# EugenHotaj/pytorch-generative

Measured on NVIDIA H100. Metric: images/sec training step (ImageGPT CIFAR-10 32x32), higher is better.
Workload: dtype bf16

## Files before the change

pytorch_generative_b200/csrc/pg_common.cuh:

```cuda
#pragma once

#include <cuda.h>
#include <cuda_bf16.h>
#include <cuda_runtime.h>
#include <stdint.h>
#include <stdio.h>

#include "../../include/pg_b200.h"

typedef __nv_bfloat16 bf16;
typedef __nv_bfloat162 bf162;

void pg_set_error(const char* fmt, ...);
int pg_check_launch(const char* what);

#define PG_REQUIRE(cond, ...)            \
  do {                                   \
    if (!(cond)) {                       \
      pg_set_error(__VA_ARGS__);         \
      return 1;                          \
    }                                    \
  } while (0)

static inline bool pg_aligned16(const void* p) { return (reinterpret_cast<uintptr_t>(p) & 15) == 0; }

#define PG_CUDA(call)                                                             \
  do {                                                                            \
    cudaError_t _e = (call);                                                      \
    if (_e != cudaSuccess) {                                                      \
      pg_set_error("%s failed: %s (%s:%d)", #call, cudaGetErrorString(_e), __FILE__, __LINE__); \
      return 1;                                                                   \
    }                                                                             \
  } while (0)

int pg_make_tmap_2d_bf16(CUtensorMap* out, const void* base, uint64_t rows, uint64_t cols,
                         uint64_t ld, uint32_t box_rows, uint32_t box_cols);
int pg_make_tmap_nd_bf16(CUtensorMap* out, const void* base, int rank, const uint64_t* dims,
                         const uint64_t* strides_bytes , const uint32_t* box,
                         int swizzle128);
int pg_make_tmap_nd(CUtensorMap* out, const void* base, int elem_bytes, int rank, const uint64_t* dims,
                    const uint64_t* strides_bytes, const uint32_t* box, int swizzle_bytes);
int pg_make_tmap_2d(CUtensorMap* out, const void* base, int elem_bytes, uint64_t rows, uint64_t cols, uint64_t ld,
                    uint32_t box_rows, uint32_t box_cols, int swizzle_bytes);
int pg_num_sms();
int pg_scratch(size_t bytes, cudaStream_t stream, float** out);
int pg_sum_partials(const float* part, int nparts, long long part_stride, int M, int N, int64_t ld_out, float* out,
                    cudaStream_t stream);

#ifdef __CUDACC__

__device__ __forceinline__ uint32_t smem_u32(const void* p) {
  return static_cast<uint32_t>(__cvta_generic_to_shared(p));
}

__device__ __forceinline__ void mbar_init(uint64_t* bar, uint32_t count) {
  asm volatile("mbarrier.init.shared::cta.b64 [%0], %1;" ::"r"(smem_u32(bar)), "r"(count) : "memory");
}
__device__ __forceinline__ void fence_barrier_init() {
  asm volatile("fence.mbarrier_init.release.cluster;" ::: "memory");
}
__device__ __forceinline__ void fence_proxy_async_smem() {
  asm volatile("fence.proxy.async.shared::cta;" ::: "memory");
}
__device__ __forceinline__ void mbar_arrive_expect_tx(uint64_t* bar, uint32_t bytes) {
  asm volatile("mbarrier.arrive.expect_tx.shared::cta.b64 _, [%0], %1;" ::"r"(smem_u32(bar)), "r"(bytes)
               : "memory");
}
__device__ __forceinline__ void mbar_arrive(uint64_t* bar) {
  asm volatile("mbarrier.arrive.shared::cta.b64 _, [%0];" ::"r"(smem_u32(bar)) : "memory");
}
__device__ __forceinline__ bool mbar_try_wait(uint64_t* bar, uint32_t parity) {
  uint32_t ok;
  asm volatile(
      "{\n\t.reg .pred p;\n\t"
      "mbarrier.try_wait.parity.shared::cta.b64 p, [%1], %2;\n\t"
      "selp.u32 %0, 1, 0, p;\n\t}"
      : "=r"(ok)
      : "r"(smem_u32(bar)), "r"(parity)
      : "memory");
  return ok != 0;
// ... 238 lines not shown
```

pytorch_generative_b200/csrc/pg_gemm.cu:

```cuda
#include <stdlib.h>
#include <string.h>

#include "../../include/pg_b200.h"
#include "pg_common.cuh"

namespace {

constexpr int BM = 128;
constexpr int BK = 64;
constexpr int A_STAGE_BYTES = BM * BK * 2;
constexpr int SMEM_LIMIT = 232448;

constexpr int MAX_CONV_TAPS = 225;
struct ConvGeom {
  int mode, H, W, C, T;
  int cslabs;
  int nbpt;
  int8_t dy[MAX_CONV_TAPS], dx[MAX_CONV_TAPS];
};

struct GemmParams {
  ConvGeom conv;
  int M, N, K;
  int num_m_blk, num_n_blk;
  int k_iters;
  int k_per_split;
  int splits;
  int stages;
  int epi_tma, epi_nbuf, epi_buf_bytes, epi_in_bytes;
  int off_old, off_res0, off_res1, off_aux, off_f32, off_pre, off_bf16;
  int epi_smem;
  int store_deriv;
  int res_bf16;
  float* a_rowsum;
  float* split_part;
  float* rowsum_part;
  pg_gemm_epilogue epi;
};

struct EpiMaps {
  CUtensorMap res0, res1, aux, out_f32, out_pre, out_bf16;
  CUtensorMap bias;
};

template <bool BWD, int ACT, int N>
__device__ __forceinline__ void act_as(float (&x)[N]) {
#pragma unroll
  for (int i = 0; i < N; ++i) x[i] = BWD ? pg_act_bwd(ACT, x[i]) : pg_act_fwd(ACT, x[i]);
}
template <bool BWD, int N>
__device__ __forceinline__ void act_n(int act, float (&x)[N]) {
  switch (act) {
    case PG_ACT_RELU: act_as<BWD, PG_ACT_RELU>(x); break;
    case PG_ACT_GELU: act_as<BWD, PG_ACT_GELU>(x); break;
    case PG_ACT_ELU: act_as<BWD, PG_ACT_ELU>(x); break;
    case PG_ACT_TANH: act_as<BWD, PG_ACT_TANH>(x); break;
    case PG_ACT_GIVEN: act_as<BWD, PG_ACT_GIVEN>(x); break;
    case PG_ACT_RELU_OUT: act_as<BWD, PG_ACT_RELU_OUT>(x); break;
    case PG_ACT_ELU_OUT: act_as<BWD, PG_ACT_ELU_OUT>(x); break;
    default: act_as<BWD, PG_ACT_NONE>(x); break;
  }
}

__device__ __forceinline__ void epilogue_row32(const GemmParams& p, int row, int col0, int ncols, bool first_split,
                                               const uint32_t (&acc)[32], float* out_f32, int64_t ld_out_f32,
                                               bool accumulate) {
  const pg_gemm_epilogue& e = p.epi;
// ... 23 lines not shown
    float* o = out_f32 + (size_t)row * ld_out_f32 + col0;
    if (accumulate) {
      for (int i = 0; i < ncols; ++i) o[i] += v[i];
    } else {
      for (int i = 0; i < ncols; ++i) o[i] = v[i];
    }
  }
  if (e.out_pre) {
    bf16* o = reinterpret_cast<bf16*>(e.out_pre) + (size_t)row * e.ld_out_pre + col0;
    float d[32];
#pragma unroll
    for (int i = 0; i < 32; ++i) d[i] = v[i];
    if (p.store_deriv) act_n<true>(e.act, d);
    for (int i = 0; i < ncols; ++i) o[i] = __float2bfloat16(d[i]);
  }
  if (e.out_bf16) {
    bf16* o = reinterpret_cast<bf16*>(e.out_bf16) + (size_t)row * e.ld_out_bf16 + col0;
    if (e.act != PG_ACT_NONE) act_n<false>(e.act, v);
    for (int i = 0; i < ncols; ++i) o[i] = __float2bfloat16(v[i]);
  }
}

constexpr int GEMM_THREADS = 384;
constexpr int XP_LD = 68;
constexpr int XP_BYTES = 64 * XP_LD * 4;
constexpr int MAX_STAGES = 8;
constexpr int MAX_EPI_BUFS = 4;
constexpr int EPI_F32_BYTES = 16 * 32 * 4;
constexpr int EPI_BF16_BYTES = 16 * 32 * 2;
constexpr int EPI_BIAS_BYTES = 128 * 4;
constexpr int PRODUCER_REGS = 56;
constexpr int CONSUMER_REGS = 224;
constexpr uint32_t XPOSE_BAR = 1;
constexpr uint32_t ROWSUM_BAR = 3;
constexpr uint32_t MMA_TURN_BAR = 4;

struct WorkItem {
  int m_blk, n_blk, ks, k0, k1;
};
__device__ __forceinline__ WorkItem work_item(const GemmParams& p, int tile) {
  WorkItem w;
  w.n_blk = tile % p.num_n_blk;
  const int rest = tile / p.num_n_blk;
  w.m_blk = rest % p.num_m_blk;
  w.ks = rest / p.num_m_blk;
  w.k0 = w.ks * p.k_per_split;
  w.k1 = min(w.k0 + p.k_per_split, p.k_iters);
  return w;
}

template <int BN, bool A_MN, bool B_MN>
__device__ __forceinline__ void consumer_mainloop(uint8_t* smem, uint64_t* full_bar, uint64_t* empty_bar, int stages,
                                                  const WorkItem& w, int& s, uint32_t& ph, float (&acc)[2][BN / 2],
                                                  int turn_bar) {
  constexpr int STAGE_BYTES = A_STAGE_BYTES + BN * BK * 2;
  const int lane = threadIdx.x & 31;
  int prev = -1;
  for (int kit = w.k0; kit < w.k1; ++kit) {
    mbar_wait(&full_bar[s], ph);
    const uint32_t a_addr = smem_u32(smem + s * STAGE_BYTES);
    const uint32_t b_addr = smem_u32(smem + s * STAGE_BYTES) + A_STAGE_BYTES;
    const uint64_t b_base = B_MN ? wgmma_desc_sw128(b_addr, BK * 128, 1024) : wgmma_desc_sw128(b_addr, 16, 1024);
    wgmma_fence();
#pragma unroll
    for (int kk = 0; kk < BK / 16; ++kk) {
#pragma unroll
      for (int sl = 0; sl < 2; ++sl) {
// ... 256 lines not shown
        if (f32_out) tma_store_3d(&tm.out_f32, buf + p.off_f32, col, row, w.ks);
        if (pre_out) tma_store_2d(&tm.out_pre, buf + p.off_pre, col, row);
        if (bf16_out) tma_store_2d(&tm.out_bf16, buf + p.off_bf16, col, row);
      }
      bulk_commit_group();
      if (has_in) {
        bulk_wait_group_read<1>();
        if (i + nb - 1 < NSUB) epi_load<BN>(p, tm, w, r, g0, i + nb - 1);
      } else if (nb == 4) {
        bulk_wait_group_read<3>();
      } else if (nb == 3) {
        bulk_wait_group_read<2>();
      } else {
        bulk_wait_group_read<1>();
      }
    }
    if (++b == nb) { b = 0; par ^= 1u; }
  }
}

template <int BN, bool A_MN, bool B_MN, int EK>
__global__ void __launch_bounds__(GEMM_THREADS, 1)
gemm_wgmma_kernel(const __grid_constant__ CUtensorMap tmA, const __grid_constant__ CUtensorMap tmB,
                  const __grid_constant__ EpiMaps tmE, const GemmParams p) {
  constexpr int STAGE_BYTES = A_STAGE_BYTES + BN * BK * 2;
  extern __shared__ uint8_t smem_raw[];
  uint8_t* smem = smem_raw + ((1024u - (smem_u32(smem_raw) & 1023u)) & 1023u);
  const int STAGES = p.stages;
  uint8_t* const epi = smem + STAGES * STAGE_BYTES;
  uint64_t* full_bar = reinterpret_cast<uint64_t*>(epi + p.epi_smem);
  uint64_t* empty_bar = full_bar + MAX_STAGES;
  uint64_t* in_bar = empty_bar + MAX_STAGES;
  uint64_t* bias_bar = in_bar + 8 * MAX_EPI_BUFS;
  float* rowsum_xch = reinterpret_cast<float*>(bias_bar + 2);

  const int warp = threadIdx.x >> 5;
  const int lane = threadIdx.x & 31;
  const bool rowsum = A_MN && p.a_rowsum != nullptr;
  const int num_tiles = p.num_m_blk * p.num_n_blk * p.splits;
  if (threadIdx.x == 0) {
    tma_prefetch_desc(&tmA);
    tma_prefetch_desc(&tmB);
    for (int i = 0; i < STAGES; ++i) {
      mbar_init(&full_bar[i], 1);
      mbar_init(&empty_bar[i], rowsum ? 6 : 4);
    }
    for (int i = 0; i < 8 * MAX_EPI_BUFS + 2; ++i) mbar_init(&in_bar[i], 1);
    fence_barrier_init();
    fence_proxy_async_smem();
  }
  __syncthreads();

  if (warp < 4) {
    setmaxnreg_dec<PRODUCER_REGS>();
    if (warp == 0) {
      int s = 0;
      uint32_t ph = 0;
      for (int tile = blockIdx.x; tile < num_tiles; tile += gridDim.x) {
        const WorkItem w = work_item(p, tile);
        const int m_blk = w.m_blk, n_blk = w.n_blk;
        for (int kit = w.k0; kit < w.k1; ++kit) {
          mbar_wait(&empty_bar[s], ph ^ 1);
          uint8_t* sA = smem + s * STAGE_BYTES;
          uint8_t* sB = sA + A_STAGE_BYTES;
          mbar_arrive_expect_tx_w(&full_bar[s], STAGE_BYTES);
          if (p.conv.mode != 0) {
            const int hw = p.conv.H * p.conv.W;
// ... 10 lines not shown
              }
            } else {
              const int t = n_blk / p.conv.nbpt, nb = n_blk - t * p.conv.nbpt;
              const int pix0 = kit * BK, n = pix0 / hw, h0 = (pix0 - n * hw) / p.conv.W;
#pragma unroll
              for (int j = 0; j < BM / 64; ++j)
                tma_load_2d_w(sA + j * (BK * 128), &tmA, &full_bar[s], m_blk * BM + j * 64, kit * BK);
#pragma unroll
              for (int j = 0; j < BN / 64; ++j)
                tma_load_4d_w(sB + j * (BK * 128), &tmB, &full_bar[s], nb * BN + j * 64, p.conv.dx[t], h0 + p.conv.dy[t], n);
            }
          } else {
            if (!A_MN) {
              tma_load_2d_w(sA, &tmA, &full_bar[s], kit * BK, m_blk * BM);
            } else {
#pragma unroll
              for (int j = 0; j < BM / 64; ++j)
                tma_load_2d_w(sA + j * (BK * 128), &tmA, &full_bar[s], m_blk * BM + j * 64, kit * BK);
            }
            if (!B_MN) {
              tma_load_2d_w(sB, &tmB, &full_bar[s], kit * BK, n_blk * BN);
            } else {
#pragma unroll
              for (int j = 0; j < BN / 64; ++j)
                tma_load_2d_w(sB + j * (BK * 128), &tmB, &full_bar[s], n_blk * BN + j * 64, kit * BK);
            }
          }
          if (++s == STAGES) { s = 0; ph ^= 1; }
        }
      }
    } else if (A_MN && (warp == 2 || warp == 3)) {
      if (rowsum) {
        const int t = (warp - 2) * 32 + lane;
        const int c = t & 15, g = t >> 4;
        const uint32_t atom = (uint32_t)(c >> 3) * (BK * 128), cc = (uint32_t)(c & 7);
        int s = 0;
        uint32_t ph = 0;
        for (int tile = blockIdx.x; tile < num_tiles; tile += gridDim.x) {
          const WorkItem w = work_item(p, tile);
          const bool mine = (w.n_blk == 0);
          float acc[8];
#pragma unroll
          for (int q = 0; q < 8; ++q) acc[q] = 0.f;
          for (int kit = w.k0; kit < w.k1; ++kit) {
            mbar_wait(&full_bar[s], ph);
            if (mine) {
              const uint8_t* sA = smem + s * STAGE_BYTES + atom;
#pragma unroll
              for (int i = 0; i < BK / 4; ++i) {
                const uint32_t k = (uint32_t)(g + 4 * i);
                const uint4 v = *reinterpret_cast<const uint4*>(sA + k * 128 + ((cc ^ (k & 7u)) << 4));
                const uint32_t ww[4] = {v.x, v.y, v.z, v.w};
#pragma unroll
                for (int j = 0; j < 4; ++j) {
                  const float2 f = unpack_bf16x2(ww[j]);
                  acc[2 * j] += f.x;
                  acc[2 * j + 1] += f.y;
                }
              }
            }
            __syncwarp();
            if (lane == 0) mbar_arrive(&empty_bar[s]);
            if (++s == STAGES) { s = 0; ph ^= 1; }
          }
          if (mine) {
#pragma unroll
            for (int q = 0; q < 8; ++q) acc[q] += __shfl_xor_sync(0xffffffffu, acc[q], 16);
            named_bar_sync(ROWSUM_BAR, 64);
            if (warp == 3 && lane < 16) {
#pragma unroll
              for (int q = 0; q < 8; ++q) rowsum_xch[lane * 8 + q] = acc[q];
            }
            named_bar_sync(ROWSUM_BAR, 64);
            if (warp == 2 && lane < 16) {
#pragma unroll
              for (int q = 0; q < 8; ++q) acc[q] += rowsum_xch[lane * 8 + q];
              const int m0 = w.m_blk * BM + c * 8;
#pragma unroll
              for (int q = 0; q < 8; ++q)
                if (m0 + q < p.M) {
                  if (p.rowsum_part) p.rowsum_part[(size_t)w.ks * p.M + m0 + q] = acc[q];
                  else p.a_rowsum[m0 + q] += acc[q];
                }
            }
          }
        }
      }
    }
  } else {
    setmaxnreg_inc<CONSUMER_REGS>();
    const int cw = (warp - 4) >> 2;
    float* const xp = reinterpret_cast<float*>(epi) + cw * 64 * XP_LD;
    float acc[2][BN / 2];
    int s = 0;
    uint32_t ph = 0;
    int i = 0;
    for (int tile = blockIdx.x; tile < num_tiles; tile += gridDim.x, ++i) {
      const WorkItem w = work_item(p, tile);
      if ((i & 1) != cw) {
        const int pos = s + (w.k1 - w.k0);
        ph ^= (uint32_t)((pos / STAGES) & 1);
        s = pos % STAGES;
        continue;
      }
      const bool has_next = tile + (int)gridDim.x < num_tiles;
      if (p.epi_tma) epi_prologue<BN>(p, tmE, w, epi_ring(p, epi, cw), i >> 1);
      if (i > 0) named_bar_sync(MMA_TURN_BAR + cw, 256);
      if (p.epi_tma) epi_bias<BN>(p, tmE, w, epi_ring(p, epi, cw));
      consumer_mainloop<BN, A_MN, B_MN>(smem, full_bar, empty_bar, STAGES, w, s, ph, acc,
                                        has_next ? (int)(MMA_TURN_BAR + (cw ^ 1)) : -1);
      if constexpr (BN <= 64) {
        if (!p.epi_tma) consumer_epilogue<BN>(p, w, acc, xp, XPOSE_BAR + cw);
      }
      if (p.epi_tma) {
        const EpiRing r = epi_ring(p, epi, cw);
        if constexpr (EK != EK_GENERIC)
// ... 85 lines not shown
    if (e.bias) t += e.bias[n];
    if (p.res_bf16) {
      if (e.res0) t += __bfloat162float(reinterpret_cast<const bf16*>(e.res0)[(size_t)m * e.ld_res + n]);
      if (e.res1) t += __bfloat162float(reinterpret_cast<const bf16*>(e.res1)[(size_t)m * e.ld_res + n]);
    } else {
      if (e.res0) t += e.res0[(size_t)m * e.ld_res + n];
      if (e.res1) t += e.res1[(size_t)m * e.ld_res + n];
    }
    if (e.out_f32) e.out_f32[(size_t)m * e.ld_out_f32 + n] = t;
    if (e.out_pre)
      reinterpret_cast<bf16*>(e.out_pre)[(size_t)m * e.ld_out_pre + n] =
          __float2bfloat16(p.store_deriv ? pg_act_bwd(e.act, t) : t);
    if (e.out_bf16) reinterpret_cast<bf16*>(e.out_bf16)[(size_t)m * e.ld_out_bf16 + n] = __float2bfloat16(pg_act_fwd(e.act, t));
  }
}

int epi_kind(const GemmParams& p) {
  const pg_gemm_epilogue& e = p.epi;
  if (!p.epi_tma || e.alpha != 1.f || p.res_bf16 || p.off_old >= 0 || p.splits > 1) return EK_GENERIC;
  const bool bias = e.bias != nullptr, f32 = e.out_f32 != nullptr, bf = e.out_bf16 != nullptr;
  const bool pre = e.out_pre != nullptr, res0 = e.res0 != nullptr, res1 = e.res1 != nullptr;
  const bool no_act = e.act == PG_ACT_NONE && !p.store_deriv;
  if (bf && !f32 && !pre && !res0 && !res1 && no_act && e.dact == PG_ACT_NONE) return bias ? EK_BIAS_BF16 : EK_PLAIN;
  if (bf && !f32 && !pre && !res0 && !res1 && no_act && e.dact == PG_ACT_GIVEN && !bias) return EK_GIVEN_BF16;
  if (bf && pre && !f32 && !res0 && !res1 && bias && e.act == PG_ACT_GELU && p.store_deriv && e.dact == PG_ACT_NONE)
    return EK_BIAS_GELU2;
  if (f32 && !bf && !pre && res0 && bias && no_act && e.dact == PG_ACT_NONE)
    return res1 ? EK_BIAS_RES2_F32 : EK_BIAS_RES_F32;
  return EK_GENERIC;
}

template <int BN, bool A_MN, bool B_MN>
int launch_tc(const void* A, int64_t lda, const void* B, int64_t ldb, GemmParams& p, cudaStream_t stream) {
  CUtensorMap tmA, tmB;
  const ConvGeom& cg = p.conv;
  auto conv_map = [&](CUtensorMap* out, const void* base, int64_t ld, int pixels_per_box) {
    const int64_t n_img = (cg.mode == 1 ? (int64_t)p.M : (int64_t)p.K) / ((int64_t)cg.H * cg.W);
    uint64_t dims[4] = {(uint64_t)cg.C, (uint64_t)cg.W, (uint64_t)cg.H, (uint64_t)n_img};
    uint64_t strides[3] = {(uint64_t)ld * 2, (uint64_t)cg.W * ld * 2, (uint64_t)cg.H * cg.W * ld * 2};
    uint32_t box[4] = {64, (uint32_t)cg.W, (uint32_t)(pixels_per_box / cg.W), 1};
    return pg_make_tmap_nd_bf16(out, base, 4, dims, strides, box, 1);
  };
  if (cg.mode == 1) {
    if (conv_map(&tmA, A, lda, BM)) return 1;
  } else if (!A_MN) {
    if (pg_make_tmap_2d_bf16(&tmA, A, p.M, p.K, lda, BM, BK)) return 1;
  } else {
    if (pg_make_tmap_2d_bf16(&tmA, A, p.K, p.M, lda, BK, 64)) return 1;
  }
  if (cg.mode == 2) {
    PG_REQUIRE(B_MN && cg.C % BN == 0, "pg_gemm_bf16_conv(wgrad): channels (%d) must be a multiple of the N tile (%d)", cg.C, BN);
    p.conv.nbpt = cg.C / BN;
    if (conv_map(&tmB, B, ldb, BK)) return 1;
  } else if (!B_MN) {
    if (pg_make_tmap_2d_bf16(&tmB, B, p.N, p.K, ldb, BN, BK)) return 1;
  } else if (cg.mode == 1) {
    if (pg_make_tmap_2d_bf16(&tmB, B, cg.C, (uint64_t)cg.T * p.N, ldb, BK, 64)) return 1;
  } else {
    if (pg_make_tmap_2d_bf16(&tmB, B, p.K, p.N, ldb, BK, 64)) return 1;
  }
  EpiMaps tmE;
  memset(&tmE, 0, sizeof(tmE));
  if (p.epi_tma) {
    const pg_gemm_epilogue& e = p.epi;
    auto f32_map = [&](CUtensorMap* out, const void* base, int64_t ld) {
      return pg_make_tmap_2d(out, base, 4, p.M, p.N, ld, 16, 32, 128);
    };
    auto bf16_map = [&](CUtensorMap* out, const void* base, int64_t ld) {
      return pg_make_tmap_2d(out, base, 2, p.M, p.N, ld, 16, 32, 64);
    };
    if (e.res0 && (p.res_bf16 ? bf16_map(&tmE.res0, e.res0, e.ld_res) : f32_map(&tmE.res0, e.res0, e.ld_res))) return 1;
    if (e.res1 && (p.res_bf16 ? bf16_map(&tmE.res1, e.res1, e.ld_res) : f32_map(&tmE.res1, e.res1, e.ld_res))) return 1;
    if (p.off_aux >= 0 && bf16_map(&tmE.aux, e.aux, e.ld_aux)) return 1;
    if (e.out_pre && bf16_map(&tmE.out_pre, e.out_pre, e.ld_out_pre)) return 1;
    if (e.out_bf16 && bf16_map(&tmE.out_bf16, e.out_bf16, e.ld_out_bf16)) return 1;
    if (e.out_f32) {
      const float* base = p.split_part ? p.split_part : e.out_f32;
      const uint64_t ld = p.split_part ? (uint64_t)p.N : (uint64_t)e.ld_out_f32;
      const uint64_t dims[3] = {(uint64_t)p.N, (uint64_t)p.M, (uint64_t)p.splits};
      const uint64_t strides[2] = {ld * 4, ld * 4 * (uint64_t)p.M};
      const uint32_t box[3] = {32, 16, 1};
      if (pg_make_tmap_nd(&tmE.out_f32, base, 4, 3, dims, strides, box, 128)) return 1;
    }
    if (e.bias) {
      const uint64_t dims[1] = {(uint64_t)p.N};
      const uint32_t box[1] = {(uint32_t)BN};
      if (pg_make_tmap_nd(&tmE.bias, e.bias, 4, 1, dims, nullptr, box, 0)) return 1;
    }
  }
  constexpr int STAGE_BYTES = A_STAGE_BYTES + BN * BK * 2;
  const int fixed = 1024  + (2 * MAX_STAGES + 8 * MAX_EPI_BUFS + 2) * 8  +
                    16 * 8 * 4 ;
  const int avail = SMEM_LIMIT - fixed;
  if (p.epi_tma) {
    const int bufs_room = (avail - 2 * EPI_BIAS_BYTES - 4 * STAGE_BYTES) / (8 * p.epi_buf_bytes);
    p.epi_nbuf = min(min(MAX_EPI_BUFS, 2 * (BN / 32)), max(2, bufs_room));
    p.epi_smem = 8 * p.epi_nbuf * p.epi_buf_bytes + 2 * EPI_BIAS_BYTES;
  } else {
    p.epi_nbuf = 0;
    p.epi_smem = 2 * XP_BYTES;
  }
  int stages = (avail - p.epi_smem) / STAGE_BYTES;
  if (stages > MAX_STAGES) stages = MAX_STAGES;
  if (stages > p.k_iters + 1) stages = p.k_iters + 1 > 2 ? p.k_iters + 1 : 2;
  PG_REQUIRE(stages >= 2, "pg_gemm_bf16: %d bytes of epilogue staging leave no room for two pipeline stages",
             p.epi_smem);
  p.stages = stages;
  const int smem_bytes = stages * STAGE_BYTES + p.epi_smem + fixed;
  auto kern = gemm_wgmma_kernel<BN, A_MN, B_MN, EK_GENERIC>;
  if constexpr (BN == 128 && !A_MN) {
    switch (epi_kind(p)) {
      case EK_PLAIN: kern = gemm_wgmma_kernel<BN, A_MN, B_MN, EK_PLAIN>; break;
      case EK_BIAS_BF16: kern = gemm_wgmma_kernel<BN, A_MN, B_MN, EK_BIAS_BF16>; break;
      case EK_BIAS_GELU2: kern = gemm_wgmma_kernel<BN, A_MN, B_MN, EK_BIAS_GELU2>; break;
      case EK_GIVEN_BF16: kern = gemm_wgmma_kernel<BN, A_MN, B_MN, EK_GIVEN_BF16>; break;
      case EK_BIAS_RES_F32: kern = gemm_wgmma_kernel<BN, A_MN, B_MN, EK_BIAS_RES_F32>; break;
      case EK_BIAS_RES2_F32: kern = gemm_wgmma_kernel<BN, A_MN, B_MN, EK_BIAS_RES2_F32>; break;
      default: break;
    }
  }
  PG_CUDA(cudaFuncSetAttribute(kern, cudaFuncAttributeMaxDynamicSharedMemorySize, smem_bytes));
  const int num_tiles = p.num_m_blk * p.num_n_blk * p.splits;
  const int grid = min(num_tiles, pg_num_sms());
  kern<<<grid, GEMM_THREADS, smem_bytes, stream>>>(tmA, tmB, tmE, p);
  if (pg_check_launch("pg_gemm_bf16(wgmma)")) return 1;
  if (p.split_part &&
      pg_sum_partials(p.split_part, p.splits, (long long)p.M * p.N, p.M, p.N, p.epi.ld_out_f32, p.epi.out_f32, stream))
    return 1;
  if (p.rowsum_part && pg_sum_partials(p.rowsum_part, p.splits, p.M, 1, p.M, p.M, p.a_rowsum, stream)) return 1;
  return 0;
}

template <bool A_MN, bool B_MN>
int dispatch_bn(const void* A, int64_t lda, const void* B, int64_t ldb, GemmParams& p, cudaStream_t stream) {
  int bn;
  if (p.N > 64) bn = 128;
  else if (p.N > 32) bn = 64;
  else bn = 32;
  if (!p.epi_tma && bn > 64) bn = 64;
  if (B_MN && bn < 64) bn = 64;
  if (p.conv.mode == 2) bn = (p.conv.C % 128 == 0 && p.epi_tma) ? 128 : 64;
  p.num_n_blk = (p.N + bn - 1) / bn;
  switch (bn) {
    case 128: return launch_tc<128, A_MN, B_MN>(A, lda, B, ldb, p, stream);
    case 64: return launch_tc<64, A_MN, B_MN>(A, lda, B, ldb, p, stream);
    default: return launch_tc<32, A_MN, B_MN>(A, lda, B, ldb, p, stream);
  }
}

}

static int gemm_entry(const void* A, int a_mn_major, int64_t lda, const void* B, int b_mn_major, int64_t ldb, int M, int N,
                      int K, int split_k, const pg_gemm_epilogue* epi, int impl, const ConvGeom* conv, void* stream_) {
  cudaStream_t stream = reinterpret_cast<cudaStream_t>(stream_);
  PG_REQUIRE(A && B && epi, "pg_gemm_bf16: null operand");
  PG_REQUIRE(M > 0 && N > 0 && K > 0, "pg_gemm_bf16: empty problem M=%d N=%d K=%d", M, N, K);
  PG_REQUIRE(lda % 8 == 0 && ldb % 8 == 0, "pg_gemm_bf16: pitches must be multiples of 8 elements (lda=%lld ldb=%lld)",
             (long long)lda, (long long)ldb);
  PG_REQUIRE(epi->out_bf16 || epi->out_pre || epi->out_f32, "pg_gemm_bf16: no output requested");
  PG_REQUIRE(epi->dact == PG_ACT_NONE || epi->aux, "pg_gemm_bf16: dact needs aux");
  if (split_k < 1) split_k = 1;
  if (split_k > 1)
// ... 38 lines not shown
    if (epi->accumulate && epi->out_f32 && p.splits == 1) { p.off_old = in; in += EPI_F32_BYTES; }
    if (epi->res0) { p.off_res0 = in; in += res_bytes; }
    if (epi->res1) { p.off_res1 = in; in += res_bytes; }
    if (aux) { p.off_aux = in; in += EPI_BF16_BYTES; }
    if (epi->out_f32) { p.off_f32 = out; out += EPI_F32_BYTES; }
    if (epi->out_pre) { p.off_pre = out; out += EPI_BF16_BYTES; }
    if (epi->out_bf16) { p.off_bf16 = out; out += EPI_BF16_BYTES; }
    p.epi_in_bytes = in;
    p.epi_buf_bytes = in > out ? in : out;
  }

  if (impl == 1) {
    p.splits = 1;
    p.k_per_split = p.k_iters;
    const int nseg = (N + 31) / 32;
    const long long total = (long long)M * nseg;
    const int threads = 128;
    const long long blocks = (total + threads - 1) / threads;
    gemm_simt_kernel<<<(unsigned)blocks, threads, 0, stream>>>(reinterpret_cast<const bf16*>(A), a_mn_major, lda,
                                                                 reinterpret_cast<const bf16*>(B), b_mn_major, ldb, p);
    return pg_check_launch("pg_gemm_bf16(simt)");
  }
  if (impl == 2) {
    PG_REQUIRE(!a_mn_major && !b_mn_major && M <= 32 && !epi->accumulate && epi->dact == PG_ACT_NONE && K % 8 == 0 &&
                   (reinterpret_cast<uintptr_t>(A) & 15) == 0 && (reinterpret_cast<uintptr_t>(B) & 15) == 0 &&
                   (size_t)M * K * 2 <= 160 * 1024,
               "pg_gemm_bf16(skinny): needs a K-major forward GEMM with M <= 32 rows (M=%d K=%d)", M, K);
    const size_t smem = (size_t)M * K * 2;
    PG_CUDA(cudaFuncSetAttribute(gemm_skinny_kernel, cudaFuncAttributeMaxDynamicSharedMemorySize, 160 * 1024));
    gemm_skinny_kernel<<<(N + 7) / 8, 256, smem, stream>>>(reinterpret_cast<const bf16*>(A), lda,
                                                           reinterpret_cast<const bf16*>(B), ldb, p);
    return pg_check_launch("pg_gemm_bf16(skinny)");
  }
  if (p.splits > 1) {
    const size_t mn = (size_t)M * N, rows = p.a_rowsum ? (size_t)M : 0;
    float* part = nullptr;
    if (pg_scratch((size_t)p.splits * (mn + rows) * sizeof(float), stream, &part)) return 1;
    p.split_part = part;
    if (p.a_rowsum) p.rowsum_part = part + (size_t)p.splits * mn;
  }
  if (!a_mn_major && !b_mn_major) return dispatch_bn<false, false>(A, lda, B, ldb, p, stream);
  if (!a_mn_major && b_mn_major) return dispatch_bn<false, true>(A, lda, B, ldb, p, stream);
  if (a_mn_major && b_mn_major) return dispatch_bn<true, true>(A, lda, B, ldb, p, stream);
  return dispatch_bn<true, false>(A, lda, B, ldb, p, stream);
}

extern "C" int pg_gemm_bf16(const void* A, int a_mn_major, int64_t lda, const void* B, int b_mn_major, int64_t ldb,
                            int M, int N, int K, int split_k, const pg_gemm_epilogue* epi, int impl, void* stream_) {
  return gemm_entry(A, a_mn_major, lda, B, b_mn_major, ldb, M, N, K, split_k, epi, impl, nullptr, stream_);
}

extern "C" int pg_gemm_bf16_conv_taps(const void* A, int64_t lda, const void* B, int64_t ldb, int M, int N, int K,
                                      int split_k, const pg_gemm_epilogue* epi, int mode, int n_img, int H, int W, int C,
                                      int n_taps, const int* dy, const int* dx, void* stream_) {
  PG_REQUIRE(mode >= PG_CONV_FWD && mode <= PG_CONV_WGRAD, "pg_gemm_bf16_conv: mode %d", mode);
  PG_REQUIRE(n_taps >= 1 && n_taps <= MAX_CONV_TAPS, "pg_gemm_bf16_conv: 1..%d taps (got %d)", MAX_CONV_TAPS, n_taps);
  PG_REQUIRE(dy && dx, "pg_gemm_bf16_conv: null tap offsets");
  PG_REQUIRE(C % 64 == 0 && W >= 1 && W <= 64 && 64 % W == 0 && ((int64_t)H * W) % 128 == 0,
             "pg_gemm_bf16_conv: needs C %% 64 == 0, W | 64 and H*W %% 128 == 0 (C=%d H=%d W=%d); use pg_tap_gather otherwise",
             C, H, W);
  const int64_t P = (int64_t)n_img * H * W;
  ConvGeom cg;
  memset(&cg, 0, sizeof(cg));
  cg.H = H; cg.W = W; cg.C = C; cg.T = n_taps;
  cg.cslabs = C / 64;
  for (int t = 0; t < n_taps; ++t) {
    PG_REQUIRE(dy[t] >= -64 && dy[t] <= 64 && dx[t] >= -64 && dx[t] <= 64, "pg_gemm_bf16_conv: tap offset out of range");
    cg.dy[t] = (int8_t)dy[t];
    cg.dx[t] = (int8_t)dx[t];
  }
  if (mode == PG_CONV_WGRAD) {
    PG_REQUIRE(K == P && N == n_taps * C, "pg_gemm_bf16_conv(wgrad): K must be N*H*W and N = taps * C");
    cg.mode = 2;
// ... 15 lines not shown
```

pytorch_generative_b200/csrc/pg_host.cu:

```cuda
#include <stdarg.h>

#include <atomic>
#include <string.h>

#include "../../include/pg_b200.h"
#include "pg_common.cuh"

static thread_local char g_err[1024] = "";

void pg_set_error(const char* fmt, ...) {
  va_list ap;
  va_start(ap, fmt);
  vsnprintf(g_err, sizeof(g_err), fmt, ap);
  va_end(ap);
}

static std::atomic<unsigned long long> g_launches{0};

int pg_check_launch(const char* what) {
  ++g_launches;
  cudaError_t e = cudaGetLastError();
  if (e != cudaSuccess) {
    pg_set_error("%s: launch failed: %s", what, cudaGetErrorString(e));
    return 1;
  }
  return 0;
}

static float* g_scratch[64] = {nullptr};
static size_t g_scratch_bytes[64] = {0};

int pg_scratch(size_t bytes, cudaStream_t stream, float** out) {
  int dev = 0;
  PG_CUDA(cudaGetDevice(&dev));
  PG_REQUIRE(dev >= 0 && dev < 64, "pg_scratch: device %d", dev);
  if (g_scratch_bytes[dev] < bytes) {
    cudaStreamCaptureStatus st = cudaStreamCaptureStatusNone;
    PG_CUDA(cudaStreamIsCapturing(stream, &st));
    PG_REQUIRE(st == cudaStreamCaptureStatusNone,
               "pg_scratch: %zu bytes of reduction scratch needed while a CUDA graph is being captured (run the step "
               "once before capturing it)", bytes);
    size_t want = 2 * g_scratch_bytes[dev];
    if (want < bytes) want = bytes;
    if (want < ((size_t)1 << 24)) want = (size_t)1 << 24;
    float* fresh = nullptr;
    PG_CUDA(cudaMalloc(&fresh, want));
    g_scratch[dev] = fresh;
    g_scratch_bytes[dev] = want;
  }
  *out = g_scratch[dev];
  return 0;
}

__global__ void sum_partials_kernel(const float* __restrict__ part, int nparts, long long part_stride, int M, int N,
                                    int64_t ld_out, float* __restrict__ out) {
  const long long total = (long long)M * N;
  for (long long i = (long long)blockIdx.x * blockDim.x + threadIdx.x; i < total; i += (long long)gridDim.x * blockDim.x) {
    float s = 0.f;
    for (int p = 0; p < nparts; ++p) s += part[p * part_stride + i];
    out[(i / N) * ld_out + i % N] += s;
  }
}
__global__ void sum_partials_warp_kernel(const float* __restrict__ part, int nparts, long long part_stride, int M, int N,
                                         int64_t ld_out, float* __restrict__ out) {
  const long long total = (long long)M * N;
  const int lane = threadIdx.x & 31;
  const long long warps = (long long)gridDim.x * (blockDim.x >> 5);
  for (long long i = ((long long)blockIdx.x * blockDim.x + threadIdx.x) >> 5; i < total; i += warps) {
    float s = 0.f;
    for (int p = lane; p < nparts; p += 32) s += part[p * part_stride + i];
    s = warp_sum(s);
    if (lane == 0) out[(i / N) * ld_out + i % N] += s;
  }
}

int pg_sum_partials(const float* part, int nparts, long long part_stride, int M, int N, int64_t ld_out, float* out,
                    cudaStream_t stream) {
  const long long total = (long long)M * N;
  const bool per_warp = nparts >= 64;
  long long blocks = ((per_warp ? total * 32 : total) + 255) / 256;
  if (blocks > (long long)pg_num_sms() * 8) blocks = (long long)pg_num_sms() * 8;
  if (blocks < 1) blocks = 1;
  if (per_warp)
    sum_partials_warp_kernel<<<(unsigned)blocks, 256, 0, stream>>>(part, nparts, part_stride, M, N, ld_out, out);
  else
    sum_partials_kernel<<<(unsigned)blocks, 256, 0, stream>>>(part, nparts, part_stride, M, N, ld_out, out);
  return pg_check_launch("pg_sum_partials");
}

extern "C" int pg_abi_version(void) { return PG_ABI_VERSION; }
extern "C" const char* pg_last_error(void) { return g_err; }

static std::atomic<int> g_reserved_sms{0};
extern "C" int pg_reserve_sms(int n) {
  const int old = g_reserved_sms.load();
  g_reserved_sms.store(n < 0 ? 0 : n);
  return old;
}

static int device_sms() {
  static int cached[64] = {0};
  int dev = 0;
  if (cudaGetDevice(&dev) != cudaSuccess || dev < 0 || dev >= 64) return 132;
  if (cached[dev] == 0) {
    int n = 0;
    if (cudaDeviceGetAttribute(&n, cudaDevAttrMultiProcessorCount, dev) != cudaSuccess || n <= 0) n = 132;
    cached[dev] = n;
  }
  return cached[dev];
}
int pg_num_sms() {
  const int n = device_sms() - g_reserved_sms.load();
  return n < 2 ? 2 : (n & ~1);
}
extern "C" int pg_sm_count(void) { return pg_num_sms(); }
extern "C" unsigned long long pg_launch_count(void) { return g_launches.load(); }

typedef CUresult (*PFN_encodeTiled)(CUtensorMap*, CUtensorMapDataType, cuuint32_t, void*, const cuuint64_t*,
                                    const cuuint64_t*, const cuuint32_t*, const cuuint32_t*,
                                    CUtensorMapInterleave, CUtensorMapSwizzle, CUtensorMapL2promotion,
// ... 66 lines not shown
```

pytorch_generative_b200/ops.py:

```python

import os

import torch
from torch.utils.weak import WeakIdKeyDictionary, WeakIdRef

from . import _lib as L

BF16 = torch.bfloat16
F32 = torch.float32

ATTN_IMPL = int(os.environ.get("PG_ATTN_IMPL", "0"))
GEMM_IMPL = int(os.environ.get("PG_GEMM_IMPL", "0"))

KERNEL_SLOTS = (64, 128)


def head_slots(dk, dv):
    def slot(d, what):
        for s in KERNEL_SLOTS:
            if d <= s:
                return s
        raise NotImplementedError(f"attention: {what}={d} channels per head exceed the widest kernel head slot "
                                  f"({KERNEL_SLOTS[-1]})")
    return slot(dk, "dk"), slot(dv, "dv")
# ... 93 lines not shown
SKINNY_ROWS = 32
SKINNY_SMEM = 160 * 1024


def linear_impl(rows, k, skinny):
    if skinny and rows <= SKINNY_ROWS and k % 8 == 0 and rows * k * 2 <= SKINNY_SMEM:
        return 2
    return GEMM_IMPL


def linear_fwd(a, w, bias=None, *, act=L.ACT_NONE, res0=None, res1=None, want_bf16=True, want_pre=False,
               want_f32=False, n_out=None, skinny=False, pre_deriv=False):
    P, K = a.shape
    n = n_out or w.shape[0]
    ob = empty((P, n), BF16, a) if want_bf16 else None
    op = empty((P, n), BF16, a) if want_pre else None
    of = empty((P, n), F32, a) if want_f32 else None
    L.gemm(a, w, P, n, K, bias=bias, res0=res0, res1=res1, out_bf16=ob, out_pre=op, out_f32=of,
           act=(act | L.ACT_STORE_DERIV) if (pre_deriv and want_pre) else act,
           impl=linear_impl(P, K, skinny))
    return ob, op, of


def linear_dgrad(dy, w, *, aux=None, dact=L.ACT_NONE, want_f32=False, k_in=None):
    P, cout = dy.shape
    cin = k_in or w.shape[1]
    ob = empty((P, cin), BF16, dy)
    of = empty((P, cin), F32, dy) if want_f32 else None
    L.gemm(dy, w[:, :cin], P, cin, min(cout, w.shape[0]), b_mn=True, aux=aux, dact=dact, out_bf16=ob, out_f32=of,
           impl=GEMM_IMPL)
    return (ob, of) if want_f32 else ob


def _split_k_for(m_out, n_out, k):
    tiles = ((m_out + 127) // 128) * ((n_out + 127) // 128)
    sms = L.sm_count()
    if os.environ.get("PG_SPLITK_ROUND_UP") == "1":
        want = max(1, (sms + tiles - 1) // tiles)
    else:
        want = max(1, sms // tiles)
    k_iters = (k + 63) // 64
    return max(1, min(want, k_iters // 8 if k_iters >= 16 else 1))


def linear_wgrad(dy, a, dw_out, db_out=None):
    P, cout = dy.shape
    cin = a.shape[1]
    assert dw_out.dtype == F32 and dw_out.shape[0] >= cout
    if db_out is not None and GEMM_IMPL != 0:
        L.colsum(dy, db_out, accumulate=True)
        db_out = None
    L.gemm(dy, a, cout, cin, P, a_mn=True, b_mn=True, out_f32=dw_out, accumulate=True,
           split_k=_split_k_for(cout, cin, P), impl=GEMM_IMPL, bias_grad=db_out)


def conv_fwd(x, wcat, bias, n_img, h, w, taps, *, act=L.ACT_NONE, res0=None, res1=None, want_bf16=True, want_pre=False,
             want_f32=False, pre_deriv=False):
    P, C = x.shape
    n = wcat.shape[0]
    ob = empty((P, n), BF16, x) if want_bf16 else None
    op = empty((P, n), BF16, x) if want_pre else None
    of = empty((P, n), F32, x) if want_f32 else None
    L.gemm_conv(x, wcat, P, n, len(taps) * C, L.CONV_FWD, n_img, h, w, C, taps, bias=bias, res0=res0, res1=res1,
                out_bf16=ob, out_pre=op, out_f32=of, act=(act | L.ACT_STORE_DERIV) if (pre_deriv and want_pre) else act)
    return ob, op, of


def conv_dgrad(dy, wcat, cin, n_img, h, w, taps, *, aux=None, dact=L.ACT_NONE, want_f32=False, want_bf16=True, res0=None):
    P, cout = dy.shape
    ob = empty((P, cin), BF16, dy) if want_bf16 else None
    of = empty((P, cin), F32, dy) if want_f32 else None
    L.gemm_conv(dy, wcat, P, cin, len(taps) * cout, L.CONV_DGRAD, n_img, h, w, cout, [(-a, -b) for a, b in taps], aux=aux,
                dact=dact, res0=res0, out_bf16=ob, out_f32=of)
    return ob, of


def conv_wgrad(dy, x, dw_out, n_img, h, w, taps, db_out=None):
    P, cout = dy.shape
    C = x.shape[1]
    T = len(taps)
    assert dw_out.dtype == F32 and dw_out.shape[0] >= cout and dw_out.shape[1] == T * C
    bn = 256 if C % 256 == 0 else (128 if C % 128 == 0 else 64)
    tiles = ((cout + 127) // 128) * (T * C // bn)
    k_iters = (P + 63) // 64
    split = max(1, min(max(1, L.sm_count() // tiles), k_iters // 8 if k_iters >= 16 else 1))
    L.gemm_conv(dy, x, cout, T * C, P, L.CONV_WGRAD, n_img, h, w, C, taps, out_f32=dw_out, accumulate=True, split_k=split,
                bias_grad=db_out)


def bias_grad(dy, out=None):
    C = dy.shape[1]
    if out is None:
        out = torch.zeros(C, dtype=F32, device=dy.device)
    L.colsum(dy, out, accumulate=True)
    return out


def layernorm_fwd(x, gamma, beta, eps, want_bf16=True, want_f32=False):
    P, C = x.shape
    yb = empty((P, C), BF16, x) if want_bf16 else None
    yf = empty((P, C), F32, x) if want_f32 else None
    mean = empty((P,), F32, x)
    rstd = empty((P,), F32, x)
    L.layernorm_fwd(x, gamma, beta, eps, y_bf16=yb, y_f32=yf, mean=mean, rstd=rstd)
    return yb, yf, mean, rstd


def layernorm_bwd(dy, x, gamma, mean, rstd, dres0=None, dres1=None, want_bf16=True, want_f32=True, want_colsum=False,
                  stats=None):
    P, ld = x.shape
    C = gamma.numel()
    dxf = empty((P, ld), F32, x) if want_f32 else None
    dxb = empty((P, ld), BF16, x) if want_bf16 else None
    if stats is None:
        stats = zeros((3, C), F32, x)
    L.layernorm_bwd(dy, x, gamma, mean, rstd, dres0=dres0, dres1=dres1, dx_f32=dxf, dx_bf16=dxb, dgamma=stats[0],
                    dbeta=stats[1], dx_colsum=stats[2] if want_colsum else None)
    if want_colsum:
# ... 18 lines not shown
```

Baseline: 547.3.

## Spread bias-grad rowsum across n-blocks and drop smem exchange in wgrad GEMM

Rewrites the fused row-sum (bias gradient) producer in the weight-gradient GEMM. Each thread now owns two rows and accumulates four k-groups separately. With split-K, the k-groups are shared across up to four n-blocks instead of all being done by n_blk 0, and the partials are reduced by a new quad-aware sum_partials kernel. The shared-memory exchange and named barrier are removed. Scratch allocation moves into launch_tc, and the split-K count is recomputed so it does not create empty splits. The aim is to remove load imbalance where one CTA per m-block did all the row-sum work, at the cost of more partial storage and a wider reduction.

```diff
diff --git a/pytorch_generative_b200/csrc/pg_common.cuh b/pytorch_generative_b200/csrc/pg_common.cuh
--- a/pytorch_generative_b200/csrc/pg_common.cuh
+++ b/pytorch_generative_b200/csrc/pg_common.cuh
@@ -46,6 +46,8 @@
 int pg_scratch(size_t bytes, cudaStream_t stream, float** out);
 int pg_sum_partials(const float* part, int nparts, long long part_stride, int M, int N, int64_t ld_out, float* out,
                     cudaStream_t stream);
+int pg_sum_partials_quads(const float* part, int nparts, long long part_stride, long long quad_stride, int M, int N,
+                          int64_t ld_out, float* out, cudaStream_t stream);
 
 #ifdef __CUDACC__
 
diff --git a/pytorch_generative_b200/csrc/pg_gemm.cu b/pytorch_generative_b200/csrc/pg_gemm.cu
--- a/pytorch_generative_b200/csrc/pg_gemm.cu
+++ b/pytorch_generative_b200/csrc/pg_gemm.cu
@@ -33,6 +33,7 @@
   int store_deriv;
   int res_bf16;
   float* a_rowsum;
+  int rowsum_shares;
   float* split_part;
   float* rowsum_part;
   pg_gemm_epilogue epi;
@@ -122,7 +123,6 @@
 constexpr int PRODUCER_REGS = 56;
 constexpr int CONSUMER_REGS = 224;
 constexpr uint32_t XPOSE_BAR = 1;
-constexpr uint32_t ROWSUM_BAR = 3;
 constexpr uint32_t MMA_TURN_BAR = 4;
 
 struct WorkItem {
@@ -445,7 +445,6 @@
   uint64_t* empty_bar = full_bar + MAX_STAGES;
   uint64_t* in_bar = empty_bar + MAX_STAGES;
   uint64_t* bias_bar = in_bar + 8 * MAX_EPI_BUFS;
-  float* rowsum_xch = reinterpret_cast<float*>(bias_bar + 2);
 
   const int warp = threadIdx.x >> 5;
   const int lane = threadIdx.x & 31;
@@ -522,30 +521,30 @@
     } else if (A_MN && (warp == 2 || warp == 3)) {
       if (rowsum) {
         const int t = (warp - 2) * 32 + lane;
-        const int c = t & 15, g = t >> 4;
-        const uint32_t atom = (uint32_t)(c >> 3) * (BK * 128), cc = (uint32_t)(c & 7);
+        const uint32_t atom = (uint32_t)(t >> 5) * (BK * 128);
+        const uint32_t mc = ((uint32_t)t >> 2) & 7u, mb = ((uint32_t)t & 3u) * 4;
+        const int shares = p.rowsum_shares;
         int s = 0;
         uint32_t ph = 0;
         for (int tile = blockIdx.x; tile < num_tiles; tile += gridDim.x) {
           const WorkItem w = work_item(p, tile);
-          const bool mine = (w.n_blk == 0);
-          float acc[8];
-#pragma unroll
-          for (int q = 0; q < 8; ++q) acc[q] = 0.f;
+          const bool mine = w.n_blk < shares;
+          float acc[4][2];
+#pragma unroll
+          for (int g = 0; g < 4; ++g) acc[g][0] = acc[g][1] = 0.f;
           for (int kit = w.k0; kit < w.k1; ++kit) {
             mbar_wait(&full_bar[s], ph);
             if (mine) {
-              const uint8_t* sA = smem + s * STAGE_BYTES + atom;
-#pragma unroll
-              for (int i = 0; i < BK / 4; ++i) {
-                const uint32_t k = (uint32_t)(g + 4 * i);
-                const uint4 v = *reinterpret_cast<const uint4*>(sA + k * 128 + ((cc ^ (k & 7u)) << 4));
-                const uint32_t ww[4] = {v.x, v.y, v.z, v.w};
-#pragma unroll
-                for (int j = 0; j < 4; ++j) {
-                  const float2 f = unpack_bf16x2(ww[j]);
-                  acc[2 * j] += f.x;
-                  acc[2 * j + 1] += f.y;
+              const uint8_t* sA = smem + s * STAGE_BYTES + atom + mb;
+#pragma unroll
+              for (int g = 0; g < 4; ++g) {
+                if (g % shares != w.n_blk) continue;
+#pragma unroll
+                for (int i = 0; i < BK / 4; ++i) {
+                  const uint32_t k = (uint32_t)(g + 4 * i);
+                  const float2 f = unpack_bf16x2(*reinterpret_cast<const uint32_t*>(sA + k * 128 + ((mc ^ (k & 7u)) << 4)));
+                  acc[g][0] += f.x;
+                  acc[g][1] += f.y;
                 }
               }
             }
@@ -554,24 +553,19 @@
             if (++s == STAGES) { s = 0; ph ^= 1; }
           }
           if (mine) {
-#pragma unroll
-            for (int q = 0; q < 8; ++q) acc[q] += __shfl_xor_sync(0xffffffffu, acc[q], 16);
-            named_bar_sync(ROWSUM_BAR, 64);
-            if (warp == 3 && lane < 16) {
-#pragma unroll
-              for (int q = 0; q < 8; ++q) rowsum_xch[lane * 8 + q] = acc[q];
-            }
-            named_bar_sync(ROWSUM_BAR, 64);
-            if (warp == 2 && lane < 16) {
-#pragma unroll
-              for (int q = 0; q < 8; ++q) acc[q] += rowsum_xch[lane * 8 + q];
-              const int m0 = w.m_blk * BM + c * 8;
-#pragma unroll
-              for (int q = 0; q < 8; ++q)
-                if (m0 + q < p.M) {
-                  if (p.rowsum_part) p.rowsum_part[(size_t)w.ks * p.M + m0 + q] = acc[q];
-                  else p.a_rowsum[m0 + q] += acc[q];
-                }
+            const int m0 = w.m_blk * BM + 2 * t;
+#pragma unroll
+            for (int j = 0; j < 2; ++j) {
+              if (m0 + j >= p.M) continue;
+              if (shares > 1) {
+#pragma unroll
+                for (int g = 0; g < 4; ++g)
+                  if (g % shares == w.n_blk) p.rowsum_part[(size_t)(w.ks * 4 + g) * p.M + m0 + j] = acc[g][j];
+              } else {
+                const float v = (acc[0][j] + acc[1][j]) + (acc[2][j] + acc[3][j]);
+                if (p.rowsum_part) p.rowsum_part[(size_t)w.ks * p.M + m0 + j] = v;
+                else p.a_rowsum[m0 + j] += v;
+              }
             }
           }
         }
@@ -723,6 +717,15 @@
 
 template <int BN, bool A_MN, bool B_MN>
 int launch_tc(const void* A, int64_t lda, const void* B, int64_t ldb, GemmParams& p, cudaStream_t stream) {
+  p.rowsum_shares = !p.a_rowsum ? 0 : p.splits > 1 ? min(p.num_n_blk, 4) : 1;
+  const size_t mn_parts = p.splits > 1 ? (size_t)p.splits * p.M * p.N : 0;
+  const size_t row_parts = p.splits > 1 && p.a_rowsum ? (size_t)p.splits * (p.rowsum_shares > 1 ? 4 : 1) * p.M : 0;
+  if (mn_parts + row_parts) {
+    float* part = nullptr;
+    if (pg_scratch((mn_parts + row_parts) * sizeof(float), stream, &part)) return 1;
+    if (mn_parts) p.split_part = part;
+    if (row_parts) p.rowsum_part = part + mn_parts;
+  }
   CUtensorMap tmA, tmB;
   const ConvGeom& cg = p.conv;
   auto conv_map = [&](CUtensorMap* out, const void* base, int64_t ld, int pixels_per_box) {
@@ -780,8 +783,7 @@
     }
   }
   constexpr int STAGE_BYTES = A_STAGE_BYTES + BN * BK * 2;
-  const int fixed = 1024  + (2 * MAX_STAGES + 8 * MAX_EPI_BUFS + 2) * 8  +
-                    16 * 8 * 4 ;
+  const int fixed = 1024  + (2 * MAX_STAGES + 8 * MAX_EPI_BUFS + 2) * 8 ;
   const int avail = SMEM_LIMIT - fixed;
   if (p.epi_tma) {
     const int bufs_room = (avail - 2 * EPI_BIAS_BYTES - 4 * STAGE_BYTES) / (8 * p.epi_buf_bytes);
@@ -818,7 +820,10 @@
   if (p.split_part &&
       pg_sum_partials(p.split_part, p.splits, (long long)p.M * p.N, p.M, p.N, p.epi.ld_out_f32, p.epi.out_f32, stream))
     return 1;
-  if (p.rowsum_part && pg_sum_partials(p.rowsum_part, p.splits, p.M, 1, p.M, p.M, p.a_rowsum, stream)) return 1;
+  if (p.rowsum_part && (p.rowsum_shares > 1
+                            ? pg_sum_partials_quads(p.rowsum_part, p.splits, 4LL * p.M, p.M, 1, p.M, p.M, p.a_rowsum, stream)
+                            : pg_sum_partials(p.rowsum_part, p.splits, p.M, 1, p.M, p.M, p.a_rowsum, stream)))
+    return 1;
   return 0;
 }
 
@@ -923,13 +928,6 @@
                                                            reinterpret_cast<const bf16*>(B), ldb, p);
     return pg_check_launch("pg_gemm_bf16(skinny)");
   }
-  if (p.splits > 1) {
-    const size_t mn = (size_t)M * N, rows = p.a_rowsum ? (size_t)M : 0;
-    float* part = nullptr;
-    if (pg_scratch((size_t)p.splits * (mn + rows) * sizeof(float), stream, &part)) return 1;
-    p.split_part = part;
-    if (p.a_rowsum) p.rowsum_part = part + (size_t)p.splits * mn;
-  }
   if (!a_mn_major && !b_mn_major) return dispatch_bn<false, false>(A, lda, B, ldb, p, stream);
   if (!a_mn_major && b_mn_major) return dispatch_bn<false, true>(A, lda, B, ldb, p, stream);
   if (a_mn_major && b_mn_major) return dispatch_bn<true, true>(A, lda, B, ldb, p, stream);
diff --git a/pytorch_generative_b200/csrc/pg_host.cu b/pytorch_generative_b200/csrc/pg_host.cu
--- a/pytorch_generative_b200/csrc/pg_host.cu
+++ b/pytorch_generative_b200/csrc/pg_host.cu
@@ -52,40 +52,51 @@
   return 0;
 }
 
-__global__ void sum_partials_kernel(const float* __restrict__ part, int nparts, long long part_stride, int M, int N,
-                                    int64_t ld_out, float* __restrict__ out) {
+__device__ __forceinline__ float partial_at(const float* __restrict__ part, long long idx, long long quad_stride) {
+  if (quad_stride == 0) return part[idx];
+  return (part[idx] + part[idx + quad_stride]) + (part[idx + 2 * quad_stride] + part[idx + 3 * quad_stride]);
+}
+
+__global__ void sum_partials_kernel(const float* __restrict__ part, int nparts, long long part_stride,
+                                    long long quad_stride, int M, int N, int64_t ld_out, float* __restrict__ out) {
   const long long total = (long long)M * N;
   for (long long i = (long long)blockIdx.x * blockDim.x + threadIdx.x; i < total; i += (long long)gridDim.x * blockDim.x) {
     float s = 0.f;
-    for (int p = 0; p < nparts; ++p) s += part[p * part_stride + i];
+    for (int p = 0; p < nparts; ++p) s += partial_at(part, p * part_stride + i, quad_stride);
     out[(i / N) * ld_out + i % N] += s;
   }
 }
-__global__ void sum_partials_warp_kernel(const float* __restrict__ part, int nparts, long long part_stride, int M, int N,
-                                         int64_t ld_out, float* __restrict__ out) {
+__global__ void sum_partials_warp_kernel(const float* __restrict__ part, int nparts, long long part_stride,
+                                         long long quad_stride, int M, int N, int64_t ld_out, float* __restrict__ out) {
   const long long total = (long long)M * N;
   const int lane = threadIdx.x & 31;
   const long long warps = (long long)gridDim.x * (blockDim.x >> 5);
   for (long long i = ((long long)blockIdx.x * blockDim.x + threadIdx.x) >> 5; i < total; i += warps) {
     float s = 0.f;
-    for (int p = lane; p < nparts; p += 32) s += part[p * part_stride + i];
+    for (int p = lane; p < nparts; p += 32) s += partial_at(part, p * part_stride + i, quad_stride);
     s = warp_sum(s);
     if (lane == 0) out[(i / N) * ld_out + i % N] += s;
   }
 }
 
-int pg_sum_partials(const float* part, int nparts, long long part_stride, int M, int N, int64_t ld_out, float* out,
-                    cudaStream_t stream) {
+int pg_sum_partials_quads(const float* part, int nparts, long long part_stride, long long quad_stride, int M, int N,
+                          int64_t ld_out, float* out, cudaStream_t stream) {
   const long long total = (long long)M * N;
   const bool per_warp = nparts >= 64;
   long long blocks = ((per_warp ? total * 32 : total) + 255) / 256;
   if (blocks > (long long)pg_num_sms() * 8) blocks = (long long)pg_num_sms() * 8;
   if (blocks < 1) blocks = 1;
   if (per_warp)
-    sum_partials_warp_kernel<<<(unsigned)blocks, 256, 0, stream>>>(part, nparts, part_stride, M, N, ld_out, out);
+    sum_partials_warp_kernel<<<(unsigned)blocks, 256, 0, stream>>>(part, nparts, part_stride, quad_stride, M, N, ld_out,
+                                                                   out);
   else
-    sum_partials_kernel<<<(unsigned)blocks, 256, 0, stream>>>(part, nparts, part_stride, M, N, ld_out, out);
+    sum_partials_kernel<<<(unsigned)blocks, 256, 0, stream>>>(part, nparts, part_stride, quad_stride, M, N, ld_out, out);
   return pg_check_launch("pg_sum_partials");
+}
+
+int pg_sum_partials(const float* part, int nparts, long long part_stride, int M, int N, int64_t ld_out, float* out,
+                    cudaStream_t stream) {
+  return pg_sum_partials_quads(part, nparts, part_stride, 0, M, N, ld_out, out, stream);
 }
 
 extern "C" int pg_abi_version(void) { return PG_ABI_VERSION; }
diff --git a/pytorch_generative_b200/ops.py b/pytorch_generative_b200/ops.py
--- a/pytorch_generative_b200/ops.py
+++ b/pytorch_generative_b200/ops.py
@@ -149,15 +149,12 @@
     return (ob, of) if want_f32 else ob
 
 
-def _split_k_for(m_out, n_out, k):
-    tiles = ((m_out + 127) // 128) * ((n_out + 127) // 128)
-    sms = L.sm_count()
-    if os.environ.get("PG_SPLITK_ROUND_UP") == "1":
-        want = max(1, (sms + tiles - 1) // tiles)
-    else:
-        want = max(1, sms // tiles)
+def _split_k_for(m_out, n_out, k, bn=128):
+    tiles = ((m_out + 127) // 128) * ((n_out + bn - 1) // bn)
     k_iters = (k + 63) // 64
-    return max(1, min(want, k_iters // 8 if k_iters >= 16 else 1))
+    split = max(1, min(max(1, L.sm_count() // tiles), k_iters // 8 if k_iters >= 16 else 1))
+    k_per = (k_iters + split - 1) // split
+    return (k_iters + k_per - 1) // k_per
 
 
 def linear_wgrad(dy, a, dw_out, db_out=None):
@@ -197,10 +194,7 @@
     C = x.shape[1]
     T = len(taps)
     assert dw_out.dtype == F32 and dw_out.shape[0] >= cout and dw_out.shape[1] == T * C
-    bn = 256 if C % 256 == 0 else (128 if C % 128 == 0 else 64)
-    tiles = ((cout + 127) // 128) * (T * C // bn)
-    k_iters = (P + 63) // 64
-    split = max(1, min(max(1, L.sm_count() // tiles), k_iters // 8 if k_iters >= 16 else 1))
+    split = _split_k_for(cout, T * C, P, 256 if C % 256 == 0 else (128 if C % 128 == 0 else 64))
     L.gemm_conv(dy, x, cout, T * C, P, L.CONV_WGRAD, n_img, h, w, C, taps, out_f32=dw_out, accumulate=True, split_k=split,
                 bias_grad=db_out)
 
```

New measurement: 562.7 (median of 6 runs). 1.03x the previous value.
